# Dao-AILab/flash-attention

Hardware: AMD Instinct MI355X
Metric: attention_fwd_tflops (higher is better)
Workload: dtype bf16; 1 GPU; BASELINE config 3: B=4 H=32 S=4096 D=128 bf16 causal, forward (flash_attn_func path, fa_fwd via C ABI); batch=4, heads=32, seqlen=4096, head_dim=128, causal=True, parallelism=replicas x1

## Files before the change

### flash-attention_amd/csrc/fa_fwd_w64.hip

```cpp
#include <cstddef>
#include <cstdio>
#include <cstdlib>
#include <type_traits>

#include "fa_device.h"
#include "fa_kernel_params.h"
#include "fa_launch.h"
#include "fa_fwd_w64_regs.h"
#define FA_W64_CLOB FA_W64_ACC_CLOBBERS
#include "fa_w64_asm.h"


#define FA_W64_AH 3
#define FA_W64_KDMA_G0 0
#define FA_W64_KDMA_GS 2
#define FA_W64_VDMA_G0 1
#define FA_W64_VDMA_GS 2

namespace fa {

template <int D> FA_DEVINL constexpr int k_swz_w(int row) { return D == 128 ? (row & 15) : ((row >> 1) & 7); }
template <int D> FA_DEVINL constexpr int v_swz_w(int row) { return D == 128 ? (row & 3) : ((row >> 1) & 1); }

#define FA_W64_MFMA(E_) (std::is_same<E_, __bf16>::value ? "v_mfma_f32_32x32x16_bf16" : "v_mfma_f32_32x32x16_f16")
constexpr int W64_Q_BASE = 128;
template <typename E, int F> FA_DEVINL void mfma_s_first(f32x16& d, u32x4 a, const f32x16& c) {
  if constexpr (std::is_same<E, __bf16>::value)
    asm volatile("v_mfma_f32_32x32x16_bf16 %0, %1, a[%c3:%c4], %2" : "=&v"(d) : "v"(a), "v"(c), "i"(W64_Q_BASE + 4 * F), "i"(W64_Q_BASE + 4 * F + 3) : FA_W64_ACC_CLOBBERS);
  else
    asm volatile("v_mfma_f32_32x32x16_f16 %0, %1, a[%c3:%c4], %2" : "=&v"(d) : "v"(a), "v"(c), "i"(W64_Q_BASE + 4 * F), "i"(W64_Q_BASE + 4 * F + 3) : FA_W64_ACC_CLOBBERS);
}
template <typename E, int F> FA_DEVINL void mfma_s_acc(f32x16& d, u32x4 a) {
  if constexpr (std::is_same<E, __bf16>::value)
    asm volatile("v_mfma_f32_32x32x16_bf16 %0, %1, a[%c2:%c3], %0" : "+v"(d) : "v"(a), "i"(W64_Q_BASE + 4 * F), "i"(W64_Q_BASE + 4 * F + 3) : FA_W64_ACC_CLOBBERS);
  else
    asm volatile("v_mfma_f32_32x32x16_f16 %0, %1, a[%c2:%c3], %0" : "+v"(d) : "v"(a), "i"(W64_Q_BASE + 4 * F), "i"(W64_Q_BASE + 4 * F + 3) : FA_W64_ACC_CLOBBERS);
}
template <typename E, int T> FA_DEVINL void mfma_o_acc(u32x4 a, u32x4 b) {
  if constexpr (std::is_same<E, __bf16>::value)
    asm volatile("v_mfma_f32_32x32x16_bf16 a[%c2:%c3], %0, %1, a[%c2:%c3]" : : "v"(a), "v"(b), "i"(16 * T), "i"(16 * T + 15) : FA_W64_ACC_CLOBBERS);
  else
    asm volatile("v_mfma_f32_32x32x16_f16 a[%c2:%c3], %0, %1, a[%c2:%c3]" : : "v"(a), "v"(b), "i"(16 * T), "i"(16 * T + 15) : FA_W64_ACC_CLOBBERS);
}
template <typename E, int D, int FEAT = 0, bool PAGED = false, bool DENSE = false>
__global__ void __launch_bounds__(256, 1) fa_fwd_w64_kernel(const FwdK p) {
  constexpr bool ALIBI = FEAT == FEAT_ALIBI;
  static_assert(!PAGED || FEAT == 0, "the paged variant serves plain attention");
  static_assert(!DENSE || (FEAT == 0 && !PAGED), "the dense variant serves plain attention on contiguous keys / values");
  constexpr bool SOFTCAP = FEAT == FEAT_CAP;
  constexpr bool DROP = FEAT == FEAT_DROP;
  constexpr bool DESC = ALIBI;
  static_assert(FEAT == 0 || FEAT == FEAT_ALIBI || FEAT == FEAT_CAP || FEAT == FEAT_DROP, "feature variants of this schedule: none, causal ALiBi, softcap, dropout");
  using T = ElemTraits<E>;
  using V8 = typename T::v8;
  constexpr int NW = 4, QB = 2, BM = NW * 64, BN = 64, CPR = D / 8;
  constexpr int ROW_BYTES = D * 2;
  constexpr int TILE_BYTES = BN * ROW_BYTES;
  constexpr int KS = D / 16;
  constexpr int DB = D / 32;
  static_assert(D == 64 || D == 128, "head dims built natively: 64, 128");
  constexpr float kLn2 = 0.6931471805599453f;

  extern __shared__ __attribute__((aligned(16))) char smem[];
  char FA_LDS* lds = (char FA_LDS*)smem;
  constexpr int STAGE_BYTES = BM * (ROW_BYTES + 16);
  constexpr int Q_OFF = (4 * TILE_BYTES > STAGE_BYTES ? 4 * TILE_BYTES : STAGE_BYTES + 1023) / 1024 * 1024;

  const int tid = threadIdx.x;
  const int lane = tid & 63;
  const int wave = __builtin_amdgcn_readfirstlane(tid >> 6);
  const int hi = lane >> 5, qi = lane & 31;

  const int d_row = lane / CPR, d_pc = lane % CPR;
  constexpr int RPD = 1024 / ROW_BYTES;

  struct Blk { int b, h, m_block, sq, sk; int64_t q_row0, k_row0, q_boff, k_boff, v_boff, o_boff; };
  const int n_virtual = p.persist_total > 0 ? p.persist_total : (int)gridDim.x;
  auto load_rc = [&]() __attribute__((always_inline)) {
#if defined(__HIP_DEVICE_COMPILE__)
    const char __attribute__((address_space(4)))* ka = (const char __attribute__((address_space(4)))*)__builtin_amdgcn_kernarg_segment_ptr();
    asm volatile("" : "+s"(ka));
    const uint32_t __attribute__((address_space(4)))* w = (const uint32_t __attribute__((address_space(4)))*)(ka + offsetof(FwdK, rc));
    W64Rc r;
    r.mul[0] = w[0]; r.mul[1] = w[1]; r.mul[2] = w[2]; r.mul[3] = w[3]; r.mul[4] = w[4]; r.shifts = w[5];
    return r;
#else
    return p.rc;
#endif
  };
  const W64Rc rc0 = load_rc();
  const int g8 = (int)(gridDim.x >> 3);
  const bool snake = p.persist_total > 0 && p.wr >= 0 && p.unit_size > 1 && g8 - fastdiv(g8, rc_get(rc0, RC_UNIT)) * p.unit_size == 0;
  auto decode_id = [&](const W64Rc& rc, int vb, int round, Blk& k) __attribute__((always_inline)) -> bool {
    if (vb >= n_virtual) return false;
    if (!DENSE && p.work_list) {
      if (!work_list_item(p.work_list, vb, p.h, p.h_k, k.b, k.h, k.m_block)) return false;
    } else {
      if (!fwd_w64_decode(p, rc, vb, snake && (round & 1), k.b, k.h, k.m_block)) return false;
    }
    return true;
  };
  auto fill_blk = [&](Blk& k) __attribute__((always_inline)) -> bool {
    k.sq = p.sq; k.sk = p.sk; k.q_row0 = 0; k.k_row0 = 0;
    if constexpr (DENSE) {
      k.q_boff = (int64_t)k.b * p.q_bs; k.k_boff = (int64_t)k.b * p.k_bs; k.v_boff = (int64_t)k.b * p.v_bs; k.o_boff = (int64_t)k.b * p.o_bs;
      return k.m_block * BM < k.sq;
    }
    const int bkv = p.kv_batch_idx ? p.kv_batch_idx[k.b] : k.b;
    k.q_boff = (int64_t)k.b * p.q_bs; k.k_boff = (int64_t)bkv * p.k_bs; k.v_boff = (int64_t)bkv * p.v_bs; k.o_boff = (int64_t)k.b * p.o_bs;
    if (p.cu_q) { const int c0 = p.cu_q[k.b]; k.sq = p.cu_q[k.b + 1] - c0; k.q_row0 = c0; k.q_boff = 0; k.o_boff = 0; }
    if (p.seqused_q) k.sq = min(k.sq, p.seqused_q[k.b]);
    if (p.cu_k) { const int c0 = p.cu_k[k.b]; k.sk = p.cu_k[k.b + 1] - c0; k.k_row0 = c0; k.k_boff = 0; k.v_boff = 0; }
    if (p.seqused_k) k.sk = min(p.seqused_k[k.b] + p.seqused_add, (p.cu_k && !PAGED) ? k.sk : p.sk);
    if (p.leftpad_k) {
      const int lp = p.leftpad_k[k.b];
      k.sk = max(0, k.sk - lp);
      k.k_row0 += lp;
    }
    if constexpr (PAGED) { k.k_boff = 0; k.v_boff = 0; k.k_row0 = 0; }
    return k.m_block * BM < k.sq;
  };
  constexpr int QDMA = (BM * ROW_BYTES) / 1024 / NW;
  auto q_srd_of = [&](const Blk& k) __attribute__((always_inline)) {
    const E* base = (const E*)p.q + k.q_boff + (k.q_row0 + (int64_t)k.m_block * BM) * p.q_rs + (int64_t)k.h * p.q_hs;
    const int rows = min(BM, k.sq - k.m_block * BM);
    const unsigned long long a = (unsigned long long)base;
    const unsigned nrec = rows > 0 ? (unsigned)(((unsigned long long)(rows - 1) * (unsigned long long)p.q_rs + D) * 2ull) : 0u;
    const unsigned lo = __builtin_amdgcn_readfirstlane((unsigned)a);
    const unsigned hi16 = __builtin_amdgcn_readfirstlane((unsigned)(a >> 32)) & 0xffffu;
    const unsigned nr = __builtin_amdgcn_readfirstlane(nrec);
    u32x4 srd = {lo, hi16, nr, 0x00020000u};
    return srd;
  };
  auto dma_q_piece = [&](const u32x4& srd, int i) __attribute__((always_inline)) {
    const int pc = wave * QDMA + i;
    const int row = pc * RPD + d_row;
    const unsigned vo = (unsigned)(row * (int)p.q_rs + ((d_pc ^ k_swz_w<D>(row)) << 3)) * 2u;
    const unsigned dst = __builtin_amdgcn_readfirstlane((unsigned)(Q_OFF + pc * 1024));
    unsigned keep;
    asm volatile("s_mov_b32 %0, m0\n\ts_mov_b32 m0, %2\n\ts_nop 0\n\tbuffer_load_dwordx4 %1, %3, 0 offen lds\n\ts_mov_b32 m0, %0"
                 : "=&s"(keep) : "v"(vo), "s"(dst), "s"(srd) : "memory");
  };
  auto dma_q = [&](const u32x4& srd) __attribute__((always_inline)) {
#pragma unroll 1
    for (int i = 0; i < QDMA; ++i) dma_q_piece(srd, i);
  };
  int q_in_lds = -1;

  constexpr int NDMA = TILE_BYTES / 1024;
  constexpr int DPW = NDMA / NW;
  unsigned koff_l[DPW], voff_l[DPW];
#pragma unroll
  for (int i = 0; i < DPW; ++i) {
    const int row = (wave * DPW + i) * RPD + d_row;
    const int kc = d_pc ^ k_swz_w<D>(row);
    const int vc = ((((d_pc >> 2) ^ v_swz_w<D>(row)) << 2) | (d_pc & 3));
    koff_l[i] = (unsigned)(row * (int)p.k_rs + kc * 8) * 2u - (unsigned)(i * 1024);
    voff_l[i] = (unsigned)(row * (int)p.v_rs + vc * 8) * 2u - (unsigned)(i * 1024);
  }
  const float thr = p.rescale_thr;
  const bool has_wl = !DENSE && p.wl >= 0;

  Blk cur_id;
  cur_id.b = 0; cur_id.h = 0; cur_id.m_block = 0;
  bool cur_ok = decode_id(rc0, (int)blockIdx.x, 0, cur_id);
  for (int vb = blockIdx.x, round = 0; vb < n_virtual; vb += gridDim.x, ++round) {
  Blk blk = cur_id, nxt;
  const bool blk_ok = cur_ok && fill_blk(blk);
  nxt.b = 0; nxt.h = 0; nxt.m_block = 0;
  const W64Rc rc = load_rc();
  const bool nxt_id_ok = p.persist_total > 0 && decode_id(rc, vb + (int)gridDim.x, round + 1, nxt);
  cur_id.b = __builtin_amdgcn_readfirstlane(nxt.b); cur_id.h = __builtin_amdgcn_readfirstlane(nxt.h); cur_id.m_block = __builtin_amdgcn_readfirstlane(nxt.m_block);
  cur_ok = nxt_id_ok;
  if (!blk_ok) continue;
  const int b = blk.b, h = blk.h, m_block = blk.m_block, sq = blk.sq, sk = blk.sk;
  const int hk = fastdiv(h, rc_get(rc, RC_HKR));
  const int64_t q_row0 = blk.q_row0, k_row0 = blk.k_row0, q_boff = blk.q_boff, k_boff = blk.k_boff, v_boff = blk.v_boff, o_boff = blk.o_boff;
  const int m0 = m_block * BM;

  const E* __restrict__ kp = (const E*)p.k + k_boff + k_row0 * p.k_rs + (int64_t)hk * p.k_hs;
  const E* __restrict__ vp = (const E*)p.v + v_boff + k_row0 * p.v_rs + (int64_t)hk * p.v_hs;
  E* __restrict__ op = (E*)p.o + o_boff + q_row0 * p.o_rs + (int64_t)h * p.o_hs;
  float* __restrict__ lsep = (!DENSE && p.cu_q) ? (p.lse + (int64_t)h * p.total_q + q_row0) : (p.lse + ((int64_t)b * p.h + h) * p.sq);

  const int shift = sk - sq;
  const int blk_last = min(m0 + BM, sq) - 1;
  int kmax = sk - 1, kmin = 0;
  if (p.wr >= 0) kmax = min(kmax, blk_last + shift + p.wr);
  if (has_wl) kmin = max(0, m0 + shift - p.wl);
  const int n_min = kmin / BN;
  const int n_max = (kmax >= kmin) ? (kmax / BN + 1) : n_min;
  const int n_tiles = n_max - n_min;
  const int n_steps = 2 * n_tiles;
  const int key_base = n_min * BN;
  auto tile_of = [&](int u) __attribute__((always_inline)) { return DESC ? n_tiles - 1 - u : u; };
  auto step_key = [&](int i) __attribute__((always_inline)) { return key_base + BN * tile_of(i >> 1) + 32 * (i & 1); };
  float slope2 = 0.f;
  if constexpr (ALIBI) slope2 = p.alibi[(int64_t)b * p.alibi_bs + h] * 1.4426950408889634f;

  const int w_row0 = m0 + wave * 64;
  const int w_row1 = min(w_row0 + 63, sq - 1);
  const bool wave_valid = w_row0 < sq;
  const int w_kmax = (p.wr >= 0) ? min(sk - 1, w_row1 + shift + p.wr) : sk - 1;
  const int w_kmin = has_wl ? max(0, w_row0 + shift - p.wl) : 0;
  const int w_full_hi = (p.wr >= 0) ? min(sk - 1, w_row0 + shift + p.wr) : sk - 1;
  const int w_full_lo = has_wl ? (w_row1 + shift - p.wl) : 0;
  int lim_hi[QB], lim_lo[QB];
#pragma unroll
  for (int qb = 0; qb < QB; ++qb) {
    const int my_row = w_row0 + 32 * qb + qi;
    lim_hi[qb] = (p.wr >= 0) ? min(sk - 1, my_row + shift + p.wr) : sk - 1;
    lim_lo[qb] = has_wl ? max(0, my_row + shift - p.wl) : 0;
  }
  auto make_srd = [&](const void* base, int64_t row_stride) __attribute__((always_inline)) {
    const unsigned long long a = (unsigned long long)base;
    const unsigned lo = __builtin_amdgcn_readfirstlane((unsigned)a);
    const unsigned hi16 = __builtin_amdgcn_readfirstlane((unsigned)(a >> 32)) & 0xffffu;
    const unsigned long long bytes = sk > 0 ? ((unsigned long long)(sk - 1) * (unsigned long long)row_stride + D) * 2ull : 0ull;
    const unsigned nrec = __builtin_amdgcn_readfirstlane((unsigned)(bytes > 0xffffffffull ? 0xffffffffull : bytes));
    u32x4 s = {lo, hi16, nrec, 0x00020000u};
    return s;
  };
  const u32x4 k_srd = make_srd(kp, p.k_rs), v_srd = make_srd(vp, p.v_rs);
  const u32x4 null_srd = {k_srd[0], k_srd[1], 0u, k_srd[3]};
  const int pg_tpp = __builtin_amdgcn_readfirstlane(PAGED ? p.page_size / BN : 1);
  const int pg_last = __builtin_amdgcn_readfirstlane(sk > 0 ? (sk - 1) / max(p.page_size, 1) : 0);
  const int* __restrict__ pg_table = p.block_table + (PAGED ? (int64_t)__builtin_amdgcn_readfirstlane(b) * p.block_table_bs : 0);
  auto page_entry = [&](int page) __attribute__((always_inline)) {
    const int pc = min(max(page, 0), pg_last);
    return __builtin_amdgcn_readfirstlane(pg_table[pc]);
  };
  const unsigned pg_bytes_k = (unsigned)__builtin_amdgcn_readfirstlane((int)(unsigned)(p.k_bs * 2)), pg_bytes_v = (unsigned)__builtin_amdgcn_readfirstlane((int)(unsigned)(p.v_bs * 2));
  const unsigned tl_bytes_k = (unsigned)__builtin_amdgcn_readfirstlane((int)(unsigned)(BN * p.k_rs * 2)), tl_bytes_v = (unsigned)__builtin_amdgcn_readfirstlane((int)(unsigned)(BN * p.v_rs * 2));
  auto uniform64 = [](const void* ptr) __attribute__((always_inline)) {
    const unsigned long long a = (unsigned long long)ptr;
    const unsigned lo = (unsigned)__builtin_amdgcn_readfirstlane((int)(unsigned)a), hi = (unsigned)__builtin_amdgcn_readfirstlane((int)(unsigned)(a >> 32));
    return ((unsigned long long)hi << 32) | (unsigned long long)lo;
  };
  const unsigned long long pg_base_k = uniform64(kp), pg_base_v = uniform64(vp);
  auto tile_srd = [&](auto isvc, int blk, int tin, int n) __attribute__((always_inline)) {
    constexpr bool ISV = decltype(isvc)::value != 0;
    const unsigned rs = (unsigned)(ISV ? p.v_rs : p.k_rs);
    const int rows = (n >= 0) ? min(BN, sk - n * BN) : 0;
    const unsigned long long a = (ISV ? pg_base_v : pg_base_k) + (unsigned long long)(unsigned)blk * (unsigned long long)(ISV ? pg_bytes_v : pg_bytes_k) + (unsigned long long)((unsigned)tin * (ISV ? tl_bytes_v : tl_bytes_k));
    const unsigned nrec = rows > 0 ? ((unsigned)(rows - 1) * rs + (unsigned)D) * 2u : 0u;
    u32x4 sd = {(unsigned)a, (unsigned)(a >> 32) & 0xffffu, nrec, 0x00020000u};
    return sd;
  };
  auto dma_pieces = [&](const u32x4& srd, const unsigned (&vo)[DPW], unsigned lds_dst) __attribute__((always_inline)) {
    unsigned keep;
    const unsigned dst = __builtin_amdgcn_readfirstlane(lds_dst);
    if constexpr (DPW == 4) {
      asm volatile("s_mov_b32 %0, m0\n\ts_mov_b32 m0, %5\n\ts_nop 0\n\t"
                   "buffer_load_dwordx4 %1, %6, 0 offen lds\n\t"
                   "buffer_load_dwordx4 %2, %6, 0 offen offset:1024 lds\n\t"
                   "buffer_load_dwordx4 %3, %6, 0 offen offset:2048 lds\n\t"
                   "buffer_load_dwordx4 %4, %6, 0 offen offset:3072 lds\n\t"
                   "s_mov_b32 m0, %0"
                   : "=&s"(keep) : "v"(vo[0]), "v"(vo[1]), "v"(vo[2]), "v"(vo[3]), "s"(dst), "s"(srd) : "memory");
    } else {
      asm volatile("s_mov_b32 %0, m0\n\ts_mov_b32 m0, %3\n\ts_nop 0\n\t"
                   "buffer_load_dwordx4 %1, %4, 0 offen lds\n\t"
                   "buffer_load_dwordx4 %2, %4, 0 offen offset:1024 lds\n\t"
                   "s_mov_b32 m0, %0"
                   : "=&s"(keep) : "v"(vo[0]), "v"(vo[DPW - 1]), "s"(dst), "s"(srd) : "memory");
    }
  };
  auto dma_tile = [&](auto isvc, int buf, int t) __attribute__((always_inline)) {
    constexpr bool ISV = decltype(isvc)::value != 0;
    const bool real = t >= 0 && t < n_tiles;
    const int64_t rs = ISV ? p.v_rs : p.k_rs;
    const unsigned lds_dst = (unsigned)((ISV ? 2 + buf : buf) * TILE_BYTES + wave * DPW * 1024);
    if constexpr (PAGED) {
      const int n = n_min + t, page = max(n, 0) / pg_tpp;
      const u32x4 sd = real ? tile_srd(isvc, page_entry(page), max(n, 0) - page * pg_tpp, n) : null_srd;
      dma_pieces(sd, ISV ? voff_l : koff_l, lds_dst);
      return;
    }
    const unsigned toff = real ? (unsigned)(n_min + t) * (unsigned)(BN * 2) * (unsigned)rs : 0u;
    unsigned vo[DPW];
#pragma unroll
    for (int i = 0; i < DPW; ++i) vo[i] = (ISV ? voff_l[i] : koff_l[i]) + toff;
    dma_pieces(real ? (ISV ? v_srd : k_srd) : null_srd, vo, lds_dst);
  };

  __syncthreads();
  if (q_in_lds != vb) dma_q(q_srd_of(blk));
  if (n_tiles > 0) dma_tile(ICw<0>{}, 0, tile_of(0));
  if (q_in_lds != vb) {
    if (n_tiles > 0) { if constexpr (DPW == 4) asm volatile("s_waitcnt vmcnt(4)" ::: "memory"); else asm volatile("s_waitcnt vmcnt(2)" ::: "memory"); }
    else lds_dma_wait_all();
  }
  {
    const float cq = SOFTCAP ? p.scale * 2.885390081777927f / p.softcap : p.scale_log2;
    u32x4 qraw[QB][KS];
#pragma unroll
    for (int qb = 0; qb < QB; ++qb)
#pragma unroll
      for (int ks = 0; ks < KS; ++ks) {
        const int qbase = Q_OFF + (wave * 64 + qb * 32 + qi) * ROW_BYTES + ((hi ^ k_swz_w<D>(qi)) << 4);
        qraw[qb][ks] = *(const u32x4 FA_LDS*)(unsigned long)(unsigned)(qbase ^ (ks << 5));
      }
    auto load_q = [&](auto qbc, auto ksc) __attribute__((always_inline)) {
      constexpr int qb = decltype(qbc)::value, ks = decltype(ksc)::value;
      const V8 raw = bitcast_u32x4<V8>(qraw[qb][ks]);
      V8 sc;
#pragma unroll
      for (int j = 0; j < 8; j += 2) {
        typedef __attribute__((ext_vector_type(2))) float f32x2;
        f32x2 pr = {(float)raw[j], (float)raw[j + 1]};
        pr *= f32x2{cq, cq};
        sc[j] = (E)pr[0]; sc[j + 1] = (E)pr[1];
      }
      acc_write_frag<W64_Q_BASE + 4 * (qb * KS + ks)>(__builtin_bit_cast(u32x4, sc));
    };
    auto load_q_all = [&](auto qbc) __attribute__((always_inline)) {
      load_q(qbc, ICw<0>{}); load_q(qbc, ICw<1>{}); load_q(qbc, ICw<2>{}); load_q(qbc, ICw<3>{});
      if constexpr (KS == 8) { load_q(qbc, ICw<4>{}); load_q(qbc, ICw<5>{}); load_q(qbc, ICw<6>{}); load_q(qbc, ICw<7>{}); }
    };
    load_q_all(ICw<0>{});
    if (n_tiles > 0) dma_tile(ICw<1>{}, 1, -1);
    load_q_all(ICw<1>{});
  }
  lds_dma_wait_all();
  __syncthreads();
  u32x4 qn_srd = null_srd;
  int qn_done = QDMA, qn_per_iter = QDMA;
  {
    q_in_lds = -1;
    if (nxt_id_ok && fill_blk(nxt)) {
      asm volatile("s_waitcnt lgkmcnt(0)" ::: "memory");
      qn_srd = q_srd_of(nxt); qn_done = 0;
      qn_per_iter = n_tiles >= QDMA ? 1 : n_tiles >= QDMA / 2 ? 2 : n_tiles >= QDMA / 4 ? 4 : QDMA;
      if (n_tiles == 0) { dma_q(qn_srd); lds_dma_wait_all(); qn_done = QDMA; }
      q_in_lds = vb + (int)gridDim.x;
    }
  }
  auto q_trickle = [&]() __attribute__((always_inline)) {
    if (qn_done < QDMA) {
#pragma unroll 1
      for (int j = 0; j < qn_per_iter; ++j) dma_q_piece(qn_srd, qn_done + j);
      qn_done += qn_per_iter;
    }
  };

  const int kbase = qi * ROW_BYTES + ((hi ^ k_swz_w<D>(qi)) << 4);
  const int tr_i = lane & 15, tr_half = (lane >> 4) & 1;
  const int tr_rr = tr_i >> 2, tr_cc = tr_i & 3;
  const int vbase = (4 * hi + tr_rr) * ROW_BYTES + (v_swz_w<D>(tr_rr) << 6) + tr_half * 32 + tr_cc * 8;
  int ka[KS], va[DB];
#pragma unroll
  for (int ks = 0; ks < KS; ++ks) ka[ks] = kbase ^ (ks << 5);
#pragma unroll
  for (int db = 0; db < DB; ++db) va[db] = vbase ^ (db << 6);

  {
    u32x4 zf = {0u, 0u, 0u, 0u};
    asm volatile("" : "+v"(zf));
    acc_zero_tuples_mfma<0>(zf, std::make_integer_sequence<int, 2 * DB>{});
  }
  float m_run[QB], l_run[QB][2], o_lag[QB];
  float thr_l[QB];
  float capc = 0.f, cap_m2c = 0.f, capoff[QB] = {0.f, 0.f};
  if constexpr (SOFTCAP) {
    capc = __builtin_bit_cast(float, __builtin_amdgcn_readfirstlane(__builtin_bit_cast(int, p.softcap * 1.4426950408889634f)));
    cap_m2c = -2.f * capc;
    capoff[0] = capc; capoff[1] = capc;
  }
  unsigned drop_kr[7] = {0u, 0u, 0u, 0u, 0u, 0u, 0u}, drop_thr = 255u, drop_row[QB] = {0u, 0u};
  if constexpr (DROP) {
    const unsigned k0_ = (unsigned)__builtin_amdgcn_readfirstlane((int)drop_bh_key(p.rng, b * p.h + h));
#pragma unroll
    for (int r = 0; r < 7; ++r) drop_kr[r] = k0_ + (unsigned)r * 0x9E3779B9u;
    drop_thr = (unsigned)__builtin_amdgcn_readfirstlane((int)p.drop_thr8);
#pragma unroll
    for (int qb = 0; qb < QB; ++qb) drop_row[qb] = (unsigned)(w_row0 + 32 * qb + qi);
  }
  constexpr float kCapTiny = 7.888609052210118e-31f;
  unsigned long long lag_mask = 0ull;
  f32x16 negm[QB];
  int arel[QB] = {0, 0};
  if constexpr (ALIBI) {
#pragma unroll
    for (int qb = 0; qb < QB; ++qb) arel[qb] = 4 * hi - (w_row0 + 32 * qb + qi) - shift;
  }
  const float ainc = slope2 * 32.f;
  f32x16 sA[QB], sB[QB];
  u32x4 pfA[QB][2], pfB[QB][2];
#pragma unroll
  for (int qb = 0; qb < QB; ++qb) {
    m_run[qb] = -INFINITY; l_run[qb][0] = 0.f; l_run[qb][1] = 0.f; o_lag[qb] = 1.f; thr_l[qb] = -INFINITY;
#pragma unroll
    for (int r = 0; r < 16; ++r) { negm[qb][r] = ALIBI ? slope2 * (float)(arel[qb] + step_key(0) + acc_row(r, 0)) : 0.f; sA[qb][r] = -INFINITY; sB[qb][r] = -INFINITY; }
#pragma unroll
    for (int t = 0; t < 2; ++t) { pfA[qb][t] = u32x4{0u, 0u, 0u, 0u}; pfB[qb][t] = u32x4{0u, 0u, 0u, 0u}; }
  }

  auto rescale = [&](auto qbc, bool grow, float tmax, f32x16& s_nxt) __attribute__((always_inline)) {
    constexpr int qb = decltype(qbc)::value;
    const float m_base = (m_run[qb] == -INFINITY) ? 0.f : m_run[qb];
    const float m_upd = grow ? (tmax + m_base) : m_run[qb];
    const float m_safe = (m_upd == -INFINITY) ? 0.f : m_upd;
    const float alpha = (grow && m_run[qb] != -INFINITY) ? fast_exp2(m_run[qb] - m_safe) : 1.f;
    const float delta = m_safe - m_base;
    m_run[qb] = m_upd;
    thr_l[qb] = grow ? thr : thr_l[qb];
    l_run[qb][0] *= alpha;
    l_run[qb][1] *= alpha;
    const float neg = -m_safe;
    if constexpr (SOFTCAP) capoff[qb] = capc - m_safe;
#pragma unroll
    for (int r = 0; r < (SOFTCAP ? 0 : 16); ++r) {
      float sv = s_nxt[r], nv = negm[qb][r];
      if constexpr (ALIBI) asm volatile("v_sub_f32 %0, %0, %2\n\tv_sub_f32 %1, %1, %2" : "+v"(sv), "+v"(nv) : "v"(delta), "v"(neg));
      else asm volatile("v_sub_f32 %0, %0, %2\n\tv_mov_b32 %1, %3" : "+v"(sv), "+v"(nv) : "v"(delta), "v"(neg));
      s_nxt[r] = sv;
      negm[qb][r] = nv;
    }
    if (lag_mask != 0ull) acc_scale_range<16 * DB * qb>(o_lag[qb], std::make_integer_sequence<int, 16 * DB>{});
    o_lag[qb] = alpha;
  };
  auto decide_and_rescale = [&](const float (&tmax)[QB], f32x16 (&s_nxt)[QB]) __attribute__((always_inline)) {
    unsigned long long grow_mask;
    asm volatile("v_cmp_gt_f32 vcc, %1, %2\n\tv_cmp_gt_f32 %0, %3, %4\n\ts_or_b64 %0, %0, vcc"
                 : "=&s"(grow_mask) : "v"(tmax[0]), "v"(thr_l[0]), "v"(tmax[1]), "v"(thr_l[1]) : "vcc");
    if (__builtin_expect((grow_mask | lag_mask) != 0ull, 0)) {
      const bool g0 = tmax[0] > thr_l[0], g1 = tmax[1] > thr_l[1];
      mfma_drain_acc();
      rescale(ICw<0>{}, g0, tmax[0], s_nxt[0]);
      rescale(ICw<1>{}, g1, tmax[1], s_nxt[1]);
      lag_mask = __builtin_amdgcn_ballot_w64(o_lag[0] != 1.f || o_lag[1] != 1.f) != 0ull ? ~0ull : 0ull;
    }
  };
  auto set_mask = [&](int i_step) __attribute__((always_inline)) {
    const int k0m = step_key(i_step);
    float ninf = -INFINITY;
    asm volatile("" : "+v"(ninf));
    static_for<QB>([&](auto mqc) __attribute__((always_inline)) {
      constexpr int mq = decltype(mqc)::value;
      float nb = (SOFTCAP || m_run[mq] == -INFINITY) ? 0.f : -m_run[mq];
      const int rel_hi = min(lim_hi[mq] - k0m - 4 * hi, 31), rel_lo = max(lim_lo[mq] - k0m - 4 * hi, 0);
      const unsigned ones = (rel_hi - rel_lo >= 31) ? 0xffffffffu : ((2u << ((rel_hi - rel_lo) & 31)) - 1u);
      unsigned bits = (rel_hi >= rel_lo) ? (ones << (rel_lo & 31)) : 0u;
      if constexpr (ALIBI) nb += slope2 * (float)(arel[mq] + k0m);
// ... 258 lines not shown
      pg_tin_k = nk % pg_tpp; pg_blk_k = page_entry(nk / pg_tpp);
      pg_page_n = nn / pg_tpp; pg_tin_n = nn - pg_page_n * pg_tpp;
    }
  };
  auto step_pair = [&](auto parc, int u, auto pmc) __attribute__((always_inline)) {
    constexpr int par = decltype(parc)::value, PM = decltype(pmc)::value;
    using M0 = ICw<(PM == 1 ? 1 : PM == 2 ? 3 : 0)>; using M1 = ICw<(PM == 1 ? 2 : PM == 2 ? 4 : 0)>;
    q_trickle();
    u32x4 kring[FA_W64_AH + 1];
    const int us = __builtin_amdgcn_readfirstlane(u);
    unsigned dst_k = (unsigned)((par ^ 1) * TILE_BYTES) + wave_dst, dst_v = (unsigned)((2 + par) * TILE_BYTES) + wave_dst;
    unsigned tk_ = (unsigned)(nmin_s + (DESC ? nts_s - 2 - us : us + 1)) * step_k, tv_ = (unsigned)(nmin_s + (DESC ? nts_s - 1 - us : us)) * step_v;
    int im32 = ((us - m_lo) | (m_hi - us)) >> 31;
    dst_k = __builtin_amdgcn_readfirstlane(dst_k); dst_v = __builtin_amdgcn_readfirstlane(dst_v);
    im32 = __builtin_amdgcn_readfirstlane(im32);
    u32x4 srd_k = k_srd, srd_v = v_srd;
    if constexpr (PAGED) {
      const int bk = __builtin_amdgcn_readfirstlane(pg_blk_k), tk = __builtin_amdgcn_readfirstlane(pg_tin_k);
      const int bv = __builtin_amdgcn_readfirstlane(pg_blk_v), tv = __builtin_amdgcn_readfirstlane(pg_tin_v);
      const int pn = __builtin_amdgcn_readfirstlane(pg_page_n), tn = __builtin_amdgcn_readfirstlane(pg_tin_n);
      srd_k = tile_srd(ICw<0>{}, bk, tk, nmin_s + us + 1);
      srd_v = tile_srd(ICw<1>{}, bv, tv, nmin_s + us);
      tk_ = 0u; tv_ = 0u;
      pg_blk_v = bk; pg_tin_v = tk;
      pg_blk_k = page_entry(pn); pg_tin_k = tn;
      const bool wrap = tn + 1 == pg_tpp;
      pg_tin_n = wrap ? 0 : tn + 1;
      pg_page_n = wrap ? pn + 1 : pn;
    }
    asm volatile("" : "+s"(tk_), "+s"(tv_), "+s"(dst_k), "+s"(dst_v), "+s"(im32));
    auto masked = [&]() __attribute__((always_inline)) { int c = im32; asm volatile("" : "+s"(c)); return c != 0; };
    if constexpr (PM != 2) { if (__builtin_expect(masked(), 0)) set_mask(2 * u); }
    fast_step(ICw<0>{}, parc, sA, sB, pfA, pfB, srd_k, koff_l, tk_, dst_k, kring, DROP ? step_key(2 * us - 1) >> 2 : 0, M0{});
    if constexpr (PM != 2) { if (__builtin_expect(masked(), 0)) set_mask(2 * u + 1); }
    fast_step(ICw<1>{}, parc, sB, sA, pfB, pfA, srd_v, voff_l, tv_, dst_v, kring, DROP ? step_key(2 * us) >> 2 : 0, M1{});
    if constexpr (PM != 2) {
      if (__builtin_expect(masked(), 0)) {
        int to_last = FEAT == 0 ? u_last - 1 - us : 1;
        asm volatile("" : "+s"(to_last));
        if (to_last != 0) clear_mask(2 * u + 2);
      }
    }
    iter_end();
  };
  auto idle_iter = [&](int u) __attribute__((always_inline)) {
    q_trickle();
    dma_tile(ICw<0>{}, (u & 1) ^ 1, tile_of(u + 1)); dma_tile(ICw<1>{}, u & 1, tile_of(u));
    iter_end();
  };
  if (n_tiles > 0) {
    const bool active = u_first <= u_last;
    const int ua = active ? (u_first & ~1) : n_tiles + 1;
    int u = 0;
#pragma unroll 1
    for (; u < ua; ++u) idle_iter(u);
    if (active) {
      pg_enter(u);
      if constexpr (ALIBI) { if (u > 0) clear_mask(2 * u); }
      if constexpr (FEAT == 0) {
        step_pair(ICw<0>{}, u, ICw<1>{}); ++u;
#pragma unroll 1
        for (;;) {
          if (u >= u_last) break;
          step_pair(ICw<1>{}, u, ICw<0>{}); ++u;
          if (u >= u_last) break;
          step_pair(ICw<0>{}, u, ICw<0>{}); ++u;
        }
        if (u & 1) step_pair(ICw<1>{}, u, ICw<2>{}); else step_pair(ICw<0>{}, u, ICw<2>{});
        ++u;
      } else {
#pragma unroll 1
        for (;;) {
          step_pair(ICw<0>{}, u, ICw<0>{}); ++u;
          if (u > u_last) break;
          step_pair(ICw<1>{}, u, ICw<0>{}); ++u;
          if (u > u_last) break;
        }
      }
    }
#pragma unroll 1
    for (; u <= n_tiles; ++u) idle_iter(u);
  }

  if (wave_valid) {
  mfma_drain_acc();
  u32x4 o_srd;
  {
    const int rows = min(BM, sq - m0);
    const unsigned long long a = (unsigned long long)(op + (int64_t)m0 * p.o_rs);
    const unsigned lo = __builtin_amdgcn_readfirstlane((unsigned)a);
    const unsigned hi16 = __builtin_amdgcn_readfirstlane((unsigned)(a >> 32)) & 0xffffu;
    const unsigned nr = __builtin_amdgcn_readfirstlane((unsigned)(((unsigned long long)(rows - 1) * (unsigned long long)p.o_rs + D) * 2ull));
    o_srd = u32x4{lo, hi16, nr, 0x00020000u};
  }
  static_for<QB>([&](auto qbc) __attribute__((always_inline)) {
    constexpr int qb = decltype(qbc)::value;
    f32x16 o_v[DB];
    static_for<DB>([&](auto dbc) __attribute__((always_inline)) {
      constexpr int db = decltype(dbc)::value;
      acc_read_tuple<16 * (qb * DB + db)>(o_v[db]);
    });
    const float l_tot = half_sum(l_run[qb][0] + l_run[qb][1]);
    const bool dead = (l_tot == 0.f) || (l_tot != l_tot);
    const float inv = (dead ? 1.f : 1.f / l_tot) * o_lag[qb] * (DROP ? p.rp_keep : 1.f);
    const int row0 = w_row0 + 32 * qb;
    if (row0 < sq) {
      {
        using V4 = typename T::v4;
        constexpr int RS = ROW_BYTES + 16, RPI = 64 / CPR;
        char FA_LDS* stage = lds + (wave * 64 + qb * 32) * RS;
#pragma unroll
        for (int db = 0; db < DB; ++db)
#pragma unroll
          for (int g = 0; g < 4; ++g) {
            V4 ov;
#pragma unroll
            for (int jj = 0; jj < 4; ++jj) ov[jj] = (E)(o_v[db][4 * g + jj] * inv);
            *reinterpret_cast<V4 FA_LDS*>(stage + qi * RS + (32 * db + 8 * g + 4 * hi) * 2) = ov;
          }
        unsigned lane_off = (unsigned)(((wave * 64 + lane / CPR) * (int)p.o_rs + (lane % CPR) * 8) * 2);
        asm volatile("" : "+v"(lane_off));
#pragma unroll
        for (int i = 0; i < 32 / RPI; ++i) {
          const u32x4 x = *reinterpret_cast<const u32x4 FA_LDS*>(stage + (i * RPI + lane / CPR) * RS + (lane % CPR) * 16);
          const unsigned soff = __builtin_amdgcn_readfirstlane((unsigned)((qb * 32 + i * RPI) * (int)p.o_rs * 2));
          asm volatile("buffer_store_dwordx4 %0, %1, %2, %3 offen" : : "v"(x), "v"(lane_off), "s"(o_srd), "s"(soff) : "memory");
        }
        asm volatile("s_waitcnt lgkmcnt(0)" ::: "memory");
      }
      const int my_row = row0 + qi;
      if (my_row < sq && hi == 0) lsep[my_row] = dead ? INFINITY : (m_run[qb] * kLn2 + __logf(l_tot));
    }
  });
  }
  }
}

template <typename E, int D, int FEAT = 0, bool PAGED = false, bool DENSE = false>
static int launch_fwd_w64_t(const FwdK& p, hipStream_t stream) {
  if constexpr (FEAT == 0 && !PAGED && !DENSE) {
    if (!p.cu_q && !p.cu_k && !p.seqused_q && !p.seqused_k && !p.leftpad_k && !p.kv_batch_idx && !p.work_list && p.wl < 0)
      return launch_fwd_w64_t<E, D, 0, false, true>(p, stream);
  }
  constexpr int STAGE = 256 * (D * 2 + 16);
  constexpr int smem = ((4 * 64 * D * 2 > STAGE ? 4 * 64 * D * 2 : STAGE + 1023) / 1024 * 1024) + 256 * D * 2;
  auto kern = fa_fwd_w64_kernel<E, D, FEAT, PAGED, DENSE>;
  static std::atomic<unsigned long long> attr_mask{0};
  if (ensure_dyn_lds(attr_mask, (const void*)kern, smem, true) != 0) return -1;
  const long long total = p.work_list ? (long long)p.work_bound * p.h : units_grid(p.n_units, p.unit_size);
  if (total <= 0) return 0;
  FwdK pp = p;
  fwd_w64_reciprocals(pp);
  long long grid = total;
  const int cus = device_cu_count();
  const bool balanced = p.wr < 0 || (p.unit_size > 1 && (cus / 8) % p.unit_size == 0);
  if (!p.work_list && cus >= 8 && total > cus && balanced && knobs().w64_persist != 0) {
    grid = cus / 8 * 8;
    pp.persist_total = (int)total;
  }
  FA_LAUNCH(kern, dim3((unsigned)grid), dim3(256), smem, stream, pp);
  if (hipGetLastError() != hipSuccess) return -1;
  LastSchedule& ls = last_schedule();
  ls.fwd_kernel = 3; ls.fwd_nw = 4; ls.fwd_feat = FEAT; ls.fwd_splits = 1; ls.fwd_list = p.work_list != nullptr; ls.d = D;
  ls.bf16 = std::is_same<E, __bf16>::value;
  if (FEAT) snprintf(ls.name, sizeof(ls.name), "fa::fa_fwd_w64_kernel<%s,%d,%s>", ls.bf16 ? "bf16" : "f16", D, FEAT == FEAT_CAP ? "softcap" : FEAT == FEAT_DROP ? "dropout" : "alibi");
  else if (PAGED) snprintf(ls.name, sizeof(ls.name), "fa::fa_fwd_w64_kernel<%s,%d,paged>", ls.bf16 ? "bf16" : "f16", D);
  else if (DENSE) snprintf(ls.name, sizeof(ls.name), "fa::fa_fwd_w64_kernel<%s,%d,dense>", ls.bf16 ? "bf16" : "f16", D);
  else snprintf(ls.name, sizeof(ls.name), "fa::fa_fwd_w64_kernel<%s,%d>", ls.bf16 ? "bf16" : "f16", D);
  return 0;
}

#ifndef FA_W64_PART
#define FA_W64_PART 0
#endif
int launch_fwd_w64_bf16(const FwdK& p, int d, hipStream_t stream);
int launch_fwd_w64_f16(const FwdK& p, int d, hipStream_t stream);
#if FA_W64_PART != 1
int launch_fwd_w64_f16(const FwdK& p, int d, hipStream_t stream) {
  if (p.rng) {
    if (d == 128) return launch_fwd_w64_t<_Float16, 128, FEAT_DROP>(p, stream);
    if (d == 64) return launch_fwd_w64_t<_Float16, 64, FEAT_DROP>(p, stream);
    return -2;
  }
  if (p.softcap > 0.f) {
    if (d == 128) return launch_fwd_w64_t<_Float16, 128, FEAT_CAP>(p, stream);
    if (d == 64) return launch_fwd_w64_t<_Float16, 64, FEAT_CAP>(p, stream);
    return -2;
  }
  if (p.alibi) {
    if (d == 128) return launch_fwd_w64_t<_Float16, 128, FEAT_ALIBI>(p, stream);
    if (d == 64) return launch_fwd_w64_t<_Float16, 64, FEAT_ALIBI>(p, stream);
    return -2;
  }
  if (p.block_table) {
    if (d == 128) return launch_fwd_w64_t<_Float16, 128, 0, true>(p, stream);
    if (d == 64) return launch_fwd_w64_t<_Float16, 64, 0, true>(p, stream);
    return -2;
  }
  if (d == 128) return launch_fwd_w64_t<_Float16, 128>(p, stream);
  if (d == 64) return launch_fwd_w64_t<_Float16, 64>(p, stream);
  return -2;
}
#endif
#if FA_W64_PART != 2
int launch_fwd_w64_bf16(const FwdK& p, int d, hipStream_t stream) {
  if (p.rng) {
    if (d == 128) return launch_fwd_w64_t<__bf16, 128, FEAT_DROP>(p, stream);
    if (d == 64) return launch_fwd_w64_t<__bf16, 64, FEAT_DROP>(p, stream);
    return -2;
  }
  if (p.softcap > 0.f) {
    if (d == 128) return launch_fwd_w64_t<__bf16, 128, FEAT_CAP>(p, stream);
    if (d == 64) return launch_fwd_w64_t<__bf16, 64, FEAT_CAP>(p, stream);
    return -2;
  }
  if (p.alibi) {
    if (d == 128) return launch_fwd_w64_t<__bf16, 128, FEAT_ALIBI>(p, stream);
    if (d == 64) return launch_fwd_w64_t<__bf16, 64, FEAT_ALIBI>(p, stream);
    return -2;
  }
  if (p.block_table) {
    if (d == 128) return launch_fwd_w64_t<__bf16, 128, 0, true>(p, stream);
    if (d == 64) return launch_fwd_w64_t<__bf16, 64, 0, true>(p, stream);
    return -2;
  }
  if (d == 128) return launch_fwd_w64_t<__bf16, 128>(p, stream);
  if (d == 64) return launch_fwd_w64_t<__bf16, 64>(p, stream);
  return -2;
// ... 17 lines not shown
```

Baseline: 1088 TFLOP/s.

## Defer output epilogue into next block's prologue to overlap O stores with Q loading

In the persistent forward kernel, the output normalisation, staging and global stores of a finished block are deferred and, for plain attention, interleaved with the next block's Q fragment reads and conversion (the seam). The output staging area moves to a separate LDS region after the first K tile so it no longer aliases K/V buffers, which lets the leading __syncthreads be dropped for the featureless path. The early second tile DMA is also skipped for FEAT==0. This aims to hide epilogue store latency and barrier cost between consecutive tiles, at the cost of more LDS, more live registers and complex ordering assumptions about LDS reuse.

```diff
diff --git a/flash-attention_amd/csrc/fa_fwd_w64.hip b/flash-attention_amd/csrc/fa_fwd_w64.hip
--- a/flash-attention_amd/csrc/fa_fwd_w64.hip
+++ b/flash-attention_amd/csrc/fa_fwd_w64.hip
@@ -24,6 +24,11 @@
 
 #define FA_W64_MFMA(E_) (std::is_same<E_, __bf16>::value ? "v_mfma_f32_32x32x16_bf16" : "v_mfma_f32_32x32x16_f16")
 constexpr int W64_Q_BASE = 128;
+template <int D> struct W64Lds {
+  static constexpr int tile = 64 * D * 2, stage = 256 * (D * 2 + 16);
+  static constexpr int q_off = ((tile + stage > 4 * tile ? tile + stage : 4 * tile) + 1023) / 1024 * 1024;
+  static constexpr int bytes = q_off + 256 * D * 2;
+};
 template <typename E, int F> FA_DEVINL void mfma_s_first(f32x16& d, u32x4 a, const f32x16& c) {
   if constexpr (std::is_same<E, __bf16>::value)
     asm volatile("v_mfma_f32_32x32x16_bf16 %0, %1, a[%c3:%c4], %2" : "=&v"(d) : "v"(a), "v"(c), "i"(W64_Q_BASE + 4 * F), "i"(W64_Q_BASE + 4 * F + 3) : FA_W64_ACC_CLOBBERS);
@@ -63,8 +68,10 @@
 
   extern __shared__ __attribute__((aligned(16))) char smem[];
   char FA_LDS* lds = (char FA_LDS*)smem;
-  constexpr int STAGE_BYTES = BM * (ROW_BYTES + 16);
-  constexpr int Q_OFF = (4 * TILE_BYTES > STAGE_BYTES ? 4 * TILE_BYTES : STAGE_BYTES + 1023) / 1024 * 1024;
+  constexpr int STAGE_OFF = TILE_BYTES, STAGE_BYTES = BM * (ROW_BYTES + 16);
+  constexpr int Q_OFF = W64Lds<D>::q_off;
+  static_assert(STAGE_OFF + STAGE_BYTES <= Q_OFF && 4 * TILE_BYTES <= Q_OFF && Q_OFF % 1024 == 0, "K/V buffers and the staging rows end below the Q block");
+  static_assert(W64Lds<D>::bytes == Q_OFF + BM * ROW_BYTES && W64Lds<D>::bytes <= 160 * 1024, "the workgroup's LDS: 160 KiB per CU");
 
   const int tid = threadIdx.x;
   const int lane = tid & 63;
@@ -161,12 +168,145 @@
   const float thr = p.rescale_thr;
   const bool has_wl = !DENSE && p.wl >= 0;
 
+  constexpr bool SEAM = FEAT == 0;
+  bool pend = false;
+  bool pend_rows = false;
+  int pend_sq = 0, pend_row0 = 0;
+  float* pend_lse = nullptr;
+  unsigned pend_o0 = 0u, pend_o1 = 0u, pend_o2 = 0u;
+  float m_run[QB] = {0.f, 0.f}, l_run[QB][2] = {{0.f, 0.f}, {0.f, 0.f}}, o_lag[QB] = {1.f, 1.f};
+  constexpr int O_RS = ROW_BYTES + 16, O_RPI = 64 / CPR, O_NST = 32 / O_RPI;
+  static_assert(O_NST == KS && O_NST == 2 * DB, "the merged sequence pairs a query block's stores with the fragments of a Q block and with the d-blocks of an O block");
+  auto o_norm = [&](int qb, float& l_tot, bool& dead) __attribute__((always_inline)) {
+    l_tot = half_sum(l_run[qb][0] + l_run[qb][1]);
+    dead = (l_tot == 0.f) || (l_tot != l_tot);
+    return (dead ? 1.f : 1.f / l_tot) * o_lag[qb] * (DROP ? p.rp_keep : 1.f);
+  };
+  auto o_stage = [&](auto qbc, auto dbc, float inv) __attribute__((always_inline)) {
+    constexpr int qb = decltype(qbc)::value, db = decltype(dbc)::value;
+    using V4 = typename T::v4;
+    f32x16 o_v;
+    acc_read_tuple<16 * (qb * DB + db)>(o_v);
+    char FA_LDS* stage = lds + STAGE_OFF + (wave * 64 + qb * 32) * O_RS;
+#pragma unroll
+    for (int g = 0; g < 4; ++g) {
+      V4 ov;
+#pragma unroll
+      for (int jj = 0; jj < 4; ++jj) ov[jj] = (E)(o_v[4 * g + jj] * inv);
+      *reinterpret_cast<V4 FA_LDS*>(stage + qi * O_RS + (32 * db + 8 * g + 4 * hi) * 2) = ov;
+    }
+  };
+  auto o_back = [&](int qb, int i) __attribute__((always_inline)) {
+    const char FA_LDS* stage = lds + STAGE_OFF + (wave * 64 + qb * 32) * O_RS;
+    return *reinterpret_cast<const u32x4 FA_LDS*>(stage + (i * O_RPI + lane / CPR) * O_RS + (lane % CPR) * 16);
+  };
+  auto o_srd = [&]() __attribute__((always_inline)) {
+    const u32x4 srd = {(unsigned)__builtin_amdgcn_readfirstlane((int)pend_o0), (unsigned)__builtin_amdgcn_readfirstlane((int)pend_o1), (unsigned)__builtin_amdgcn_readfirstlane((int)pend_o2), 0x00020000u};
+    return srd;
+  };
+  auto o_store = [&](const u32x4& srd, const u32x4& x, unsigned& off, unsigned step) __attribute__((always_inline)) {
+    asm volatile("buffer_store_dwordx4 %0, %1, %2, 0 offen\n\ts_nop 0" : : "v"(x), "v"(off), "s"(srd) : "memory");
+    off += step;
+  };
+  auto o_lane_off = [&](int qb) __attribute__((always_inline)) {
+    unsigned lane_off = (unsigned)(((wave * 64 + qb * 32 + lane / CPR) * (int)p.o_rs + (lane % CPR) * 8) * 2);
+    asm volatile("" : "+v"(lane_off));
+    return lane_off;
+  };
+  auto o_step = [&]() __attribute__((always_inline)) {
+    unsigned step = (unsigned)(O_RPI * (int)p.o_rs * 2);
+    asm volatile("" : "+v"(step));
+    return step;
+  };
+  auto o_lse = [&](int qb, float l_tot, bool dead) __attribute__((always_inline)) {
+    const int my_row = pend_row0 + 32 * qb + qi;
+    if (my_row < pend_sq && hi == 0) pend_lse[my_row] = dead ? INFINITY : (m_run[qb] * kLn2 + __logf(l_tot));
+  };
+  auto epilogue = [&]() __attribute__((always_inline)) {
+    mfma_drain_acc();
+    const u32x4 srd = o_srd();
+    static_for<QB>([&](auto qbc) __attribute__((always_inline)) {
+      constexpr int qb = decltype(qbc)::value;
+      float l_tot; bool dead;
+      const float inv = o_norm(qb, l_tot, dead);
+      if (pend_row0 + 32 * qb < pend_sq) {
+        static_for<DB>([&](auto dbc) __attribute__((always_inline)) { o_stage(qbc, dbc, inv); });
+        unsigned off = o_lane_off(qb);
+        const unsigned step = o_step();
+#pragma unroll
+        for (int i = 0; i < O_NST; ++i) o_store(srd, o_back(qb, i), off, step);
+        o_lse(qb, l_tot, dead);
+      }
+    });
+  };
+  auto q_reads = [&](u32x4 (&qraw)[QB][KS]) __attribute__((always_inline)) {
+    int qrow = Q_OFF + (wave * 64 + qi) * ROW_BYTES + ((hi ^ k_swz_w<D>(qi)) << 4);
+    asm volatile("" : "+v"(qrow));
+#pragma unroll
+    for (int qb = 0; qb < QB; ++qb)
+#pragma unroll
+      for (int ks = 0; ks < KS; ++ks)
+        qraw[qb][ks] = *(const u32x4 FA_LDS*)(unsigned long)(unsigned)((qrow ^ (ks << 5)) + qb * 32 * ROW_BYTES);
+  };
+  auto q_conv = [&](auto qbc, auto ksc, const u32x4 (&qraw)[QB][KS]) __attribute__((always_inline)) {
+    constexpr int qb = decltype(qbc)::value, ks = decltype(ksc)::value;
+    const float cq = SOFTCAP ? p.scale * 2.885390081777927f / p.softcap : p.scale_log2;
+    const V8 raw = bitcast_u32x4<V8>(qraw[qb][ks]);
+    V8 sc;
+#pragma unroll
+    for (int j = 0; j < 8; j += 2) {
+      typedef __attribute__((ext_vector_type(2))) float f32x2;
+      f32x2 pr = {(float)raw[j], (float)raw[j + 1]};
+      pr *= f32x2{cq, cq};
+      sc[j] = (E)pr[0]; sc[j + 1] = (E)pr[1];
+    }
+    acc_write_frag<W64_Q_BASE + 4 * (qb * KS + ks)>(__builtin_bit_cast(u32x4, sc));
+  };
+  auto seam = [&]() __attribute__((always_inline)) {
+    mfma_drain_acc();
+    const u32x4 srd = o_srd();
+    u32x4 qraw[QB][KS], x[O_NST];
+    q_reads(qraw);
+    float lt0, lt1; bool dead0, dead1;
+    const float inv0 = o_norm(0, lt0, dead0), inv1 = o_norm(1, lt1, dead1);
+    unsigned off = o_lane_off(0);
+    const unsigned step = o_step();
+    static_for<DB>([&](auto dbc) __attribute__((always_inline)) { o_stage(ICw<0>{}, dbc, inv0); });
+    o_lse(0, lt0, dead0);
+#pragma unroll
+    for (int i = 0; i < O_NST; ++i) x[i] = o_back(0, i);
+    __builtin_amdgcn_sched_barrier(0);
+    static_for<DB>([&](auto dbc) __attribute__((always_inline)) {
+      constexpr int db = decltype(dbc)::value;
+      o_store(srd, x[2 * db], off, step);
+      o_store(srd, x[2 * db + 1], off, step);
+      o_stage(ICw<1>{}, dbc, inv1);
+      __builtin_amdgcn_sched_barrier(0);
+    });
+    o_lse(1, lt1, dead1);
+#pragma unroll
+    for (int i = 0; i < O_NST; ++i) x[i] = o_back(1, i);
+    __builtin_amdgcn_sched_barrier(0);
+    static_for<KS>([&](auto ksc) __attribute__((always_inline)) {
+      constexpr int ks = decltype(ksc)::value;
+      o_store(srd, x[ks], off, step);
+      q_conv(ICw<0>{}, ksc, qraw);
+      __builtin_amdgcn_sched_barrier(0);
+    });
+    static_for<KS>([&](auto ksc) __attribute__((always_inline)) { q_conv(ICw<1>{}, ksc, qraw); });
+  };
+
   Blk cur_id;
   cur_id.b = 0; cur_id.h = 0; cur_id.m_block = 0;
   bool cur_ok = decode_id(rc0, (int)blockIdx.x, 0, cur_id);
-  for (int vb = blockIdx.x, round = 0; vb < n_virtual; vb += gridDim.x, ++round) {
+  for (int vb = blockIdx.x, round = 0;; vb += gridDim.x, ++round) {
+  const bool have = vb < n_virtual;
   Blk blk = cur_id, nxt;
-  const bool blk_ok = cur_ok && fill_blk(blk);
+  const bool blk_ok = have && cur_ok && fill_blk(blk);
+  const bool merge = SEAM && pend && blk_ok && q_in_lds == vb && pend_row0 + 32 < pend_sq;
+  if (pend && pend_rows && !merge) epilogue();
+  pend = false;
+  if (!have) break;
   nxt.b = 0; nxt.h = 0; nxt.m_block = 0;
   const W64Rc rc = load_rc();
   const bool nxt_id_ok = p.persist_total > 0 && decode_id(rc, vb + (int)gridDim.x, round + 1, nxt);
@@ -284,43 +424,21 @@
     dma_pieces(real ? (ISV ? v_srd : k_srd) : null_srd, vo, lds_dst);
   };
 
-  __syncthreads();
+  if constexpr (FEAT != 0) __syncthreads();
   if (q_in_lds != vb) dma_q(q_srd_of(blk));
   if (n_tiles > 0) dma_tile(ICw<0>{}, 0, tile_of(0));
   if (q_in_lds != vb) {
     if (n_tiles > 0) { if constexpr (DPW == 4) asm volatile("s_waitcnt vmcnt(4)" ::: "memory"); else asm volatile("s_waitcnt vmcnt(2)" ::: "memory"); }
     else lds_dma_wait_all();
   }
-  {
-    const float cq = SOFTCAP ? p.scale * 2.885390081777927f / p.softcap : p.scale_log2;
+  if (merge) {
+    seam();
+  } else {
     u32x4 qraw[QB][KS];
-#pragma unroll
-    for (int qb = 0; qb < QB; ++qb)
-#pragma unroll
-      for (int ks = 0; ks < KS; ++ks) {
-        const int qbase = Q_OFF + (wave * 64 + qb * 32 + qi) * ROW_BYTES + ((hi ^ k_swz_w<D>(qi)) << 4);
-        qraw[qb][ks] = *(const u32x4 FA_LDS*)(unsigned long)(unsigned)(qbase ^ (ks << 5));
-      }
-    auto load_q = [&](auto qbc, auto ksc) __attribute__((always_inline)) {
-      constexpr int qb = decltype(qbc)::value, ks = decltype(ksc)::value;
-      const V8 raw = bitcast_u32x4<V8>(qraw[qb][ks]);
-      V8 sc;
-#pragma unroll
-      for (int j = 0; j < 8; j += 2) {
-        typedef __attribute__((ext_vector_type(2))) float f32x2;
-        f32x2 pr = {(float)raw[j], (float)raw[j + 1]};
-        pr *= f32x2{cq, cq};
-        sc[j] = (E)pr[0]; sc[j + 1] = (E)pr[1];
-      }
-      acc_write_frag<W64_Q_BASE + 4 * (qb * KS + ks)>(__builtin_bit_cast(u32x4, sc));
-    };
-    auto load_q_all = [&](auto qbc) __attribute__((always_inline)) {
-      load_q(qbc, ICw<0>{}); load_q(qbc, ICw<1>{}); load_q(qbc, ICw<2>{}); load_q(qbc, ICw<3>{});
-      if constexpr (KS == 8) { load_q(qbc, ICw<4>{}); load_q(qbc, ICw<5>{}); load_q(qbc, ICw<6>{}); load_q(qbc, ICw<7>{}); }
-    };
-    load_q_all(ICw<0>{});
-    if (n_tiles > 0) dma_tile(ICw<1>{}, 1, -1);
-    load_q_all(ICw<1>{});
+    q_reads(qraw);
+    static_for<KS>([&](auto ksc) __attribute__((always_inline)) { q_conv(ICw<0>{}, ksc, qraw); });
+    if constexpr (FEAT != 0) { if (n_tiles > 0) dma_tile(ICw<1>{}, 1, -1); }
+    static_for<KS>([&](auto ksc) __attribute__((always_inline)) { q_conv(ICw<1>{}, ksc, qraw); });
   }
   lds_dma_wait_all();
   __syncthreads();
@@ -359,7 +477,6 @@
     asm volatile("" : "+v"(zf));
     acc_zero_tuples_mfma<0>(zf, std::make_integer_sequence<int, 2 * DB>{});
   }
-  float m_run[QB], l_run[QB][2], o_lag[QB];
   float thr_l[QB];
   float capc = 0.f, cap_m2c = 0.f, capoff[QB] = {0.f, 0.f};
   if constexpr (SOFTCAP) {
@@ -784,56 +901,14 @@
     for (; u <= n_tiles; ++u) idle_iter(u);
   }
 
-  if (wave_valid) {
-  mfma_drain_acc();
-  u32x4 o_srd;
   {
     const int rows = min(BM, sq - m0);
     const unsigned long long a = (unsigned long long)(op + (int64_t)m0 * p.o_rs);
     const unsigned lo = __builtin_amdgcn_readfirstlane((unsigned)a);
     const unsigned hi16 = __builtin_amdgcn_readfirstlane((unsigned)(a >> 32)) & 0xffffu;
     const unsigned nr = __builtin_amdgcn_readfirstlane((unsigned)(((unsigned long long)(rows - 1) * (unsigned long long)p.o_rs + D) * 2ull));
-    o_srd = u32x4{lo, hi16, nr, 0x00020000u};
-  }
-  static_for<QB>([&](auto qbc) __attribute__((always_inline)) {
-    constexpr int qb = decltype(qbc)::value;
-    f32x16 o_v[DB];
-    static_for<DB>([&](auto dbc) __attribute__((always_inline)) {
-      constexpr int db = decltype(dbc)::value;
-      acc_read_tuple<16 * (qb * DB + db)>(o_v[db]);
-    });
-    const float l_tot = half_sum(l_run[qb][0] + l_run[qb][1]);
-    const bool dead = (l_tot == 0.f) || (l_tot != l_tot);
-    const float inv = (dead ? 1.f : 1.f / l_tot) * o_lag[qb] * (DROP ? p.rp_keep : 1.f);
-    const int row0 = w_row0 + 32 * qb;
-    if (row0 < sq) {
-      {
-        using V4 = typename T::v4;
-        constexpr int RS = ROW_BYTES + 16, RPI = 64 / CPR;
-        char FA_LDS* stage = lds + (wave * 64 + qb * 32) * RS;
-#pragma unroll
-        for (int db = 0; db < DB; ++db)
-#pragma unroll
-          for (int g = 0; g < 4; ++g) {
-            V4 ov;
-#pragma unroll
-            for (int jj = 0; jj < 4; ++jj) ov[jj] = (E)(o_v[db][4 * g + jj] * inv);
-            *reinterpret_cast<V4 FA_LDS*>(stage + qi * RS + (32 * db + 8 * g + 4 * hi) * 2) = ov;
-          }
-        unsigned lane_off = (unsigned)(((wave * 64 + lane / CPR) * (int)p.o_rs + (lane % CPR) * 8) * 2);
-        asm volatile("" : "+v"(lane_off));
-#pragma unroll
-        for (int i = 0; i < 32 / RPI; ++i) {
-          const u32x4 x = *reinterpret_cast<const u32x4 FA_LDS*>(stage + (i * RPI + lane / CPR) * RS + (lane % CPR) * 16);
-          const unsigned soff = __builtin_amdgcn_readfirstlane((unsigned)((qb * 32 + i * RPI) * (int)p.o_rs * 2));
-          asm volatile("buffer_store_dwordx4 %0, %1, %2, %3 offen" : : "v"(x), "v"(lane_off), "s"(o_srd), "s"(soff) : "memory");
-        }
-        asm volatile("s_waitcnt lgkmcnt(0)" ::: "memory");
-      }
-      const int my_row = row0 + qi;
-      if (my_row < sq && hi == 0) lsep[my_row] = dead ? INFINITY : (m_run[qb] * kLn2 + __logf(l_tot));
-    }
-  });
+    pend_o0 = lo; pend_o1 = hi16; pend_o2 = nr;
+    pend = true; pend_rows = wave_valid; pend_sq = sq; pend_row0 = w_row0; pend_lse = lsep;
   }
   }
 }
@@ -844,8 +919,7 @@
     if (!p.cu_q && !p.cu_k && !p.seqused_q && !p.seqused_k && !p.leftpad_k && !p.kv_batch_idx && !p.work_list && p.wl < 0)
       return launch_fwd_w64_t<E, D, 0, false, true>(p, stream);
   }
-  constexpr int STAGE = 256 * (D * 2 + 16);
-  constexpr int smem = ((4 * 64 * D * 2 > STAGE ? 4 * 64 * D * 2 : STAGE + 1023) / 1024 * 1024) + 256 * D * 2;
+  constexpr int smem = W64Lds<D>::bytes;
   auto kern = fa_fwd_w64_kernel<E, D, FEAT, PAGED, DENSE>;
   static std::atomic<unsigned long long> attr_mask{0};
   if (ensure_dyn_lds(attr_mask, (const void*)kern, smem, true) != 0) return -1;
```

After: 1091 TFLOP/s, median of 6. Within noise of the previous version (+0.3%).
